# craston/object_detection_cib

Hardware: AMD Instinct MI355X
Metric: images/sec YOLOv5s 640px train (higher is better)
Workload: dtype bf16; 1 GPU; yv5s coco-zipf-like synthetic, 640px, bf16 storage/fp32 accumulate, batch 64/GPU, fwd+assign+loss+bwd+SGD, targets 4-30 boxes/img; global_batch=64, parallelism=dp1, launch=hipGraph replay, collectives=none, launcher=none, attempt=0

## Files before the change

### object_detection_cib_amd/csrc/conv_wgrad.hip

```cpp
#include <stdlib.h>

#include "kodhip_common.h"

namespace {

struct WgradArgs {
  const bf16_t* x;
  const bf16_t* dy;
  float* part;
  int B, Hs, Ws, ldx, xcoff, Cin;
  int Ho, Wo, M;
  int N, K, Kp;
  int KH, KW, SH, SW, PH, PW;
  int ldy, ycoff;
  int m_per_split, splits;
  int tiles_n, tiles_k;
  uint32_t magic_cin, magic_kw;
  uint32_t magic_hwo, magic_wo;
  const bf16_t* dy2;
  int n_half;
  int linear_map;
};

__device__ __forceinline__ bool wg_map(const WgradArgs& a, int bid, int tiles, int& tile, int& split) {
// ... 138 lines not shown
    if (st + 1 < nsteps) load_tile(m_begin + (st + 1) * 32);
    const unsigned char* Ys = lds + buf * STAGE;
    const unsigned char* Xs = Ys + 32 * SY;
#pragma unroll
    for (int ks = 0; ks < 2; ++ks) {
      bf16x8 yf[RN], xf[RK];
#pragma unroll
      for (int i = 0; i < RN; ++i) {
        const unsigned char* p = Ys + (ks * 16 + tr_row) * SY + ((wn * RN + i) * 32 + tr_col) * 2;
        s16x4 lo = __builtin_amdgcn_ds_read_tr16_b64_v4i16((s16x4 __attribute__((address_space(3)))*)(p));
        s16x4 hi = __builtin_amdgcn_ds_read_tr16_b64_v4i16((s16x4 __attribute__((address_space(3)))*)(p + 4 * SY));
        typedef short s16x8 __attribute__((ext_vector_type(8)));
        s16x8 t = {lo[0], lo[1], lo[2], lo[3], hi[0], hi[1], hi[2], hi[3]};
        yf[i] = __builtin_bit_cast(bf16x8, t);
      }
#pragma unroll
      for (int jj = 0; jj < RK; ++jj) {
        const unsigned char* p = Xs + (ks * 16 + tr_row) * SX + ((wk * RK + jj) * 32 + tr_col) * 2;
        s16x4 lo = __builtin_amdgcn_ds_read_tr16_b64_v4i16((s16x4 __attribute__((address_space(3)))*)(p));
        s16x4 hi = __builtin_amdgcn_ds_read_tr16_b64_v4i16((s16x4 __attribute__((address_space(3)))*)(p + 4 * SX));
        typedef short s16x8 __attribute__((ext_vector_type(8)));
        s16x8 t = {lo[0], lo[1], lo[2], lo[3], hi[0], hi[1], hi[2], hi[3]};
        xf[jj] = __builtin_bit_cast(bf16x8, t);
      }
#pragma unroll
      for (int i = 0; i < RN; ++i)
#pragma unroll
        for (int jj = 0; jj < RK; ++jj)
          acc[i][jj] = __builtin_amdgcn_mfma_f32_32x32x16_bf16(yf[i], xf[jj], acc[i][jj], 0, 0, 0);
    }
    if (st + 1 < nsteps) store_tile(buf ^ 1);
    __syncthreads();
  }

  float* slab = a.part + (size_t)split * a.N * a.Kp;
#pragma unroll
  for (int i = 0; i < RN; ++i)
#pragma unroll
    for (int jj = 0; jj < RK; ++jj) {
      int k = k0 + (wk * RK + jj) * 32 + (lane & 31);
#pragma unroll
      for (int e = 0; e < 16; ++e) {
        int n = n0 + (wn * RN + i) * 32 + 8 * (e >> 2) + 4 * (lane >> 5) + (e & 3);
        if (n < a.N && k < a.Kp) slab[(size_t)n * a.Kp + k] = acc[i][jj][e];
      }
    }
}

__host__ __device__ constexpr int swz_mask(int row_b) { return row_b % 256 == 0 ? 3 : (row_b % 128 == 0 ? 2 : 0); }
__device__ __forceinline__ int swz(int row, int mask) { return mask == 3 ? 4 * (row & 3) : (mask == 2 ? 4 * ((row >> 1) & 1) : 0); }

template <int N>
__device__ __forceinline__ void wait_vm() { asm volatile("s_waitcnt vmcnt(%0)" ::"n"(N) : "memory"); }
template <int WN, int WK, int RN, int RK, int NST, int RS, int GM>
__global__ __launch_bounds__(64 * WN * WK) void conv_wgrad_dma_kernel(WgradArgs a, uint32_t x_bytes, uint32_t dy_bytes) {
  constexpr int NW = WN * WK;
  constexpr int TNB = WN * RN * 32;
  constexpr int TKB = WK * RK * 32;
  constexpr int RBY = TNB * 2, RBX = TKB * 2;
  constexpr int NIY = RS * RBY / 1024, NIX = RS * RBX / 1024;
  constexpr int KS = RS / 16;
  constexpr int NI = NIY + NIX;
  constexpr int SLOTS = (NI + NW - 1) / NW;
  constexpr int STAGE = RS * RBY + RS * RBX;
  constexpr int MY = swz_mask(RBY), MX = swz_mask(RBX);
  static_assert((RS * RBY) % 1024 == 0 && (RS * RBX) % 1024 == 0, "tile rows must fill whole DMA instructions");
  __shared__ __attribute__((aligned(1024))) unsigned char lds[NST * STAGE];

  const int tid = threadIdx.x;
  const int lane = tid & 63;
  const int wave = __builtin_amdgcn_readfirstlane(tid >> 6);
  const int wn = wave / WK, wk = wave % WK;

  const int bid = blockIdx.x;
  const int tiles = a.tiles_n * a.tiles_k;
  int tile, split;
  if (!wg_map(a, bid, tiles, tile, split)) return;
  const int nt = tile % a.tiles_n;
  const bool half2 = a.n_half && nt >= (a.tiles_n >> 1);
  const int n0 = half2 ? a.n_half + (nt - (a.tiles_n >> 1)) * TNB : nt * TNB;
  const int ny0 = half2 ? n0 - a.n_half : n0;
  const int ny_hi = a.n_half ? a.n_half : a.N;
  const int n_hi = (a.n_half && !half2) ? a.n_half : a.N;
  const int k0 = (tile / a.tiles_n) * TKB;
  const int m_begin = split * a.m_per_split;
  int m_end = m_begin + a.m_per_split;
  if (m_end > a.M) m_end = a.M;
  const int HWo = a.Ho * a.Wo;

#if defined(__HIP_DEVICE_COMPILE__)
  __amdgpu_buffer_rsrc_t rs_x = __builtin_amdgcn_make_buffer_rsrc((void*)a.x, 0, x_bytes, 0x00020000);
  __amdgpu_buffer_rsrc_t rs_y = __builtin_amdgcn_make_buffer_rsrc((void*)(half2 ? a.dy2 : a.dy), 0, dy_bytes, 0x00020000);
#endif

  int s_row[SLOTS];
  uint32_t s_off[SLOTS];
  bool s_ok[SLOTS];
  int s_cy[SLOTS], s_cx[SLOTS];
  int my_slots = 0;
  constexpr bool pointwise = GM == 1;
  constexpr bool ROLE_STATIC = (NIY % NW == 0) && (NI % NW == 0);
#pragma unroll
  for (int i = 0; i < SLOTS; ++i) {
    const int t = wave + i * NW;
    s_row[i] = 0; s_off[i] = 0; s_ok[i] = false; s_cy[i] = s_cx[i] = 0;
    if (!ROLE_STATIC && t >= NI) continue;
    ++my_slots;
    if (ROLE_STATIC ? (i < NIY / NW) : (t < NIY)) {
      const int L = t * 1024 + lane * 16;
      const int row = L / RBY, pc = (L % RBY) >> 4;
      const int c = pc ^ swz(row, MY);
      s_row[i] = row;
      s_ok[i] = (ny0 + c * 8) < ny_hi;
      s_off[i] = (uint32_t)(((long)(m_begin + row) * a.ldy + a.ycoff + ny0 + c * 8) * 2);
    } else {
      const int L = (t - NIY) * 1024 + lane * 16;
      const int row = L / RBX, pc = (L % RBX) >> 4;
      const int c = pc ^ swz(row, MX);
      const int k = k0 + c * 8;
      const uint32_t tap = __umulhi((uint32_t)k, a.magic_cin);
      const int ci = k - (int)tap * a.Cin;
      const int kh = (a.KW == 1) ? (int)tap : (int)__umulhi(tap, a.magic_kw);
      s_row[i] = row;
      s_ok[i] = k < a.K;
      s_cy[i] = kh - a.PH; s_cx[i] = ((int)tap - kh * a.KW) - a.PW;
      s_off[i] = (uint32_t)((a.xcoff + ci) * 2);
      if (pointwise) s_off[i] = (uint32_t)(((long)(m_begin + row) * a.ldx + a.xcoff + ci) * 2);
    }
  }
  const uint32_t magic_hwo = a.magic_hwo, magic_wo = a.magic_wo;
  const uint32_t ldx2 = (uint32_t)a.ldx * 2u, ystep = (uint32_t)(RS * a.ldy * 2), xstep = (uint32_t)(RS * a.ldx * 2);

  int issued = 0;
  auto issue = [&](int stage) {
    unsigned char* Ys = lds + stage * STAGE;
    const int mb = m_begin + issued * RS;
#pragma unroll
    for (int i = 0; i < SLOTS; ++i) {
      const int t = wave + i * NW;
      if (!ROLE_STATIC && t >= NI) continue;
      const int m = mb + s_row[i];
      uint32_t vo;
      bool ok = s_ok[i] && m < m_end;
      const bool is_y = ROLE_STATIC ? (i < NIY / NW) : (t < NIY);
      if (is_y) {
        vo = s_off[i];
        s_off[i] += ystep;
      } else if (pointwise) {
        vo = s_off[i];
        s_off[i] += xstep;
      } else {
        uint32_t b = magic_hwo ? __umulhi((uint32_t)m, magic_hwo) : (uint32_t)m;
        int rem = m - (int)b * HWo;
        if (rem < 0) { rem += HWo; --b; }
        uint32_t oy = magic_wo ? __umulhi((uint32_t)rem, magic_wo) : (uint32_t)rem;
        int ox = rem - (int)oy * a.Wo;
        if (ox < 0) { ox += a.Wo; --oy; }
        const int iy = (int)oy * a.SH + s_cy[i];
        const int ix = ox * a.SW + s_cx[i];
        ok = ok && (unsigned)iy < (unsigned)a.Hs && (unsigned)ix < (unsigned)a.Ws;
        vo = (((uint32_t)b * (uint32_t)a.Hs + (uint32_t)iy) * (uint32_t)a.Ws + (uint32_t)ix) * ldx2 + s_off[i];
      }
      vo = ok ? vo : 0xFFFFFFF0u;
#if defined(__HIP_DEVICE_COMPILE__) && !defined(WG_ABL_NODMA)
      if (is_y)
        __builtin_amdgcn_raw_ptr_buffer_load_lds(rs_y, (__attribute__((address_space(3))) void*)(Ys + t * 1024), 16, vo, 0, 0, 0);
      else
        __builtin_amdgcn_raw_ptr_buffer_load_lds(rs_x, (__attribute__((address_space(3))) void*)(Ys + t * 1024), 16, vo, 0, 0, 0);
#else
      (void)vo; (void)Ys;
#endif
    }
    ++issued;
  };

  f32x16 acc[RN][RK];
#pragma unroll
  for (int i = 0; i < RN; ++i)
#pragma unroll
    for (int jj = 0; jj < RK; ++jj)
#pragma unroll
      for (int e = 0; e < 16; ++e) acc[i][jj][e] = 0.f;

  const int tr_row = 8 * (lane >> 5) + ((lane & 15) >> 2);
  const int tr_col = 16 * ((lane >> 4) & 1) + 4 * (lane & 3);
  const int sy = swz(tr_row, MY), sx = swz(tr_row, MX);
  const uint32_t lds_base = (uint32_t)(uintptr_t)(__attribute__((address_space(3))) unsigned char*)lds;
  uint32_t yoff[RN], xoff[RK];
#pragma unroll
  for (int i = 0; i < RN; ++i) {
    const int col = (wn * RN + i) * 32 + tr_col;
    yoff[i] = (uint32_t)(tr_row * RBY + (((col >> 3) ^ sy) << 4) + (col & 7) * 2);
  }
#pragma unroll
  for (int jj = 0; jj < RK; ++jj) {
    const int col = (wk * RK + jj) * 32 + tr_col;
    xoff[jj] = (uint32_t)(tr_row * RBX + (((col >> 3) ^ sx) << 4) + (col & 7) * 2);
  }

  const int nsteps = (m_end - m_begin + RS - 1) / RS;
#pragma unroll
  for (int p = 0; p < NST - 1; ++p)
    if (p < nsteps) issue(p);
  for (int st = 0; st < nsteps; ++st) {
    const int newer = nsteps - 1 - st;
    if (newer >= NST - 2) {
      if (my_slots == SLOTS) wait_vm<(NST - 2) * SLOTS>(); else wait_vm<(NST - 2) * (SLOTS - 1)>();
    } else if (newer == 1 && NST > 3) {
      if (my_slots == SLOTS) wait_vm<SLOTS>(); else wait_vm<SLOTS - 1>();
    } else {
      wait_vm<0>();
    }
    __builtin_amdgcn_s_barrier();
#ifndef WG_ABL_NOISSUE
    if (st + NST - 1 < nsteps) issue((st + NST - 1) % NST);
#endif
    const uint32_t ys = lds_base + (uint32_t)((st % NST) * STAGE);
    const uint32_t xs = ys + RS * RBY;
    s16x4 ylo[KS][RN], yhi[KS][RN], xlo[KS][RK], xhi[KS][RK];
#pragma unroll
    for (int ks = 0; ks < KS; ++ks) {
#pragma unroll
      for (int i = 0; i < RN; ++i) {
        const uint32_t p = ys + yoff[i] + (uint32_t)(ks * 16 * RBY);
        asm volatile("ds_read_b64_tr_b16 %0, %1" : "=v"(ylo[ks][i]) : "v"(p) : "memory");
        asm volatile("ds_read_b64_tr_b16 %0, %1" : "=v"(yhi[ks][i]) : "v"(p + 4 * RBY) : "memory");
      }
#pragma unroll
      for (int jj = 0; jj < RK; ++jj) {
        const uint32_t p = xs + xoff[jj] + (uint32_t)(ks * 16 * RBX);
        asm volatile("ds_read_b64_tr_b16 %0, %1" : "=v"(xlo[ks][jj]) : "v"(p) : "memory");
        asm volatile("ds_read_b64_tr_b16 %0, %1" : "=v"(xhi[ks][jj]) : "v"(p + 4 * RBX) : "memory");
      }
    }
#pragma unroll
    for (int ks = 0; ks < KS; ++ks) {
      constexpr int PER = 2 * (RN + RK);
      if (ks == KS - 1) asm volatile("s_waitcnt lgkmcnt(0)" ::: "memory");
      else if ((KS - 1 - ks) * PER >= 15) asm volatile("s_waitcnt lgkmcnt(15)" ::: "memory");
      else if (ks == KS - 2) asm volatile("s_waitcnt lgkmcnt(%0)" ::"n"(PER < 15 ? PER : 15) : "memory");
      else asm volatile("s_waitcnt lgkmcnt(%0)" ::"n"(2 * PER < 15 ? 2 * PER : 15) : "memory");
#pragma unroll
      for (int i = 0; i < RN; ++i) asm volatile("" : "+v"(ylo[ks][i]), "+v"(yhi[ks][i]));
#pragma unroll
      for (int jj = 0; jj < RK; ++jj) asm volatile("" : "+v"(xlo[ks][jj]), "+v"(xhi[ks][jj]));
      typedef short s16x8 __attribute__((ext_vector_type(8)));
      bf16x8 yf[RN], xf[RK];
#pragma unroll
      for (int i = 0; i < RN; ++i) {
        s16x8 t = {ylo[ks][i][0], ylo[ks][i][1], ylo[ks][i][2], ylo[ks][i][3], yhi[ks][i][0], yhi[ks][i][1], yhi[ks][i][2], yhi[ks][i][3]};
        yf[i] = __builtin_bit_cast(bf16x8, t);
      }
#pragma unroll
      for (int jj = 0; jj < RK; ++jj) {
        s16x8 t = {xlo[ks][jj][0], xlo[ks][jj][1], xlo[ks][jj][2], xlo[ks][jj][3], xhi[ks][jj][0], xhi[ks][jj][1], xhi[ks][jj][2], xhi[ks][jj][3]};
        xf[jj] = __builtin_bit_cast(bf16x8, t);
      }
#pragma unroll
      for (int i = 0; i < RN; ++i)
#pragma unroll
        for (int jj = 0; jj < RK; ++jj)
#ifdef WG_ABL_NOMFMA
          asm volatile("" ::"v"(yf[i]), "v"(xf[jj]));
#else
          acc[i][jj] = __builtin_amdgcn_mfma_f32_32x32x16_bf16(yf[i], xf[jj], acc[i][jj], 0, 0, 0);
#endif
    }
  }
  float* slab = a.part + (size_t)split * a.N * a.Kp;
#pragma unroll
  for (int i = 0; i < RN; ++i)
#pragma unroll
    for (int jj = 0; jj < RK; ++jj) {
      int k = k0 + (wk * RK + jj) * 32 + (lane & 31);
#pragma unroll
      for (int e = 0; e < 16; ++e) {
        int n = n0 + (wn * RN + i) * 32 + 8 * (e >> 2) + 4 * (lane >> 5) + (e & 3);
        if (n < n_hi && k < a.Kp) slab[(size_t)n * a.Kp + k] = acc[i][jj][e];
      }
    }
}

template <int WN, int RN, int WC, int NST>
__global__ __launch_bounds__(64 * WN * 3 * WC) void conv_wgrad_row3_kernel(WgradArgs a, uint32_t x_bytes, uint32_t dy_bytes) {
  constexpr int RS = 32;
  constexpr int NW = WN * 3 * WC;
  constexpr int TNB = WN * RN * 32;
  constexpr int RBY = TNB * 2;
  constexpr int RBX = 64;
  constexpr int XR = 48;
  constexpr int NIY = RS * RBY / 1024;
  constexpr int NXT = 3 * WC;
  constexpr int NIX = NXT * 3;
  constexpr int NI = NIY + NIX;
  constexpr int SLOTS = (NI + NW - 1) / NW;
  constexpr int XT_BYTES = XR * RBX;
  constexpr int STAGE = RS * RBY + NXT * XT_BYTES;
  constexpr int MY = swz_mask(RBY);
  constexpr int KS = RS / 16;
  static_assert((RS * RBY) % 1024 == 0 && XT_BYTES % 1024 == 0, "tiles must fill whole DMA instructions");
  __shared__ __attribute__((aligned(1024))) unsigned char lds[NST * STAGE];

  const int tid = threadIdx.x;
  const int lane = tid & 63;
  const int wave = __builtin_amdgcn_readfirstlane(tid >> 6);
  const int wc = wave % WC, kh = (wave / WC) % 3, wn = wave / (3 * WC);

  const int bid = blockIdx.x;
  const int tiles = a.tiles_n * a.tiles_k;
  int tile, split;
  if (!wg_map(a, bid, tiles, tile, split)) return;
  const int n0 = (tile % a.tiles_n) * TNB;
  const int c0 = (tile / a.tiles_n) * (WC * 32);
  const int m_begin = split * a.m_per_split;
  int m_end = m_begin + a.m_per_split;
  if (m_end > a.M) m_end = a.M;
  const int W = a.Ws, H = a.Hs, HW = a.Hs * a.Ws, BHW = a.B * HW;

#if defined(__HIP_DEVICE_COMPILE__)
  __amdgpu_buffer_rsrc_t rs_x = __builtin_amdgcn_make_buffer_rsrc((void*)a.x, 0, x_bytes, 0x00020000);
// ... 142 lines not shown
#pragma unroll
      for (int i = 0; i < RN; ++i) asm volatile("" : "+v"(ylo[ks][i]), "+v"(yhi[ks][i]));
#pragma unroll
      for (int kw = 0; kw < 3; ++kw) asm volatile("" : "+v"(xlo[ks][kw]), "+v"(xhi[ks][kw]));
      typedef short s16x8 __attribute__((ext_vector_type(8)));
      typedef unsigned int u32x2 __attribute__((ext_vector_type(2)));
      if ((inv0 | inv2) != 0) {
        const int sh = ks * 16 + 8 * (lane >> 5);
#pragma unroll
        for (int side = 0; side < 2; ++side) {
          const uint32_t bits = ((side == 0 ? inv0 : inv2) >> sh) & 0xFFu;
          const int kw = side == 0 ? 0 : 2;
          u32x2 lo = __builtin_bit_cast(u32x2, xlo[ks][kw]), hi = __builtin_bit_cast(u32x2, xhi[ks][kw]);
          lo[0] &= ((bits & 1u) ? 0u : 0xFFFFu) | ((bits & 2u) ? 0u : 0xFFFF0000u);
          lo[1] &= ((bits & 4u) ? 0u : 0xFFFFu) | ((bits & 8u) ? 0u : 0xFFFF0000u);
          hi[0] &= ((bits & 16u) ? 0u : 0xFFFFu) | ((bits & 32u) ? 0u : 0xFFFF0000u);
          hi[1] &= ((bits & 64u) ? 0u : 0xFFFFu) | ((bits & 128u) ? 0u : 0xFFFF0000u);
          xlo[ks][kw] = __builtin_bit_cast(s16x4, lo); xhi[ks][kw] = __builtin_bit_cast(s16x4, hi);
        }
      }
      bf16x8 yf[RN], xf[3];
#pragma unroll
      for (int i = 0; i < RN; ++i) {
        s16x8 t = {ylo[ks][i][0], ylo[ks][i][1], ylo[ks][i][2], ylo[ks][i][3], yhi[ks][i][0], yhi[ks][i][1], yhi[ks][i][2], yhi[ks][i][3]};
        yf[i] = __builtin_bit_cast(bf16x8, t);
      }
#pragma unroll
      for (int kw = 0; kw < 3; ++kw) {
        s16x8 t = {xlo[ks][kw][0], xlo[ks][kw][1], xlo[ks][kw][2], xlo[ks][kw][3], xhi[ks][kw][0], xhi[ks][kw][1], xhi[ks][kw][2], xhi[ks][kw][3]};
        xf[kw] = __builtin_bit_cast(bf16x8, t);
      }
#pragma unroll
      for (int i = 0; i < RN; ++i)
#pragma unroll
        for (int kw = 0; kw < 3; ++kw)
          acc[i][kw] = __builtin_amdgcn_mfma_f32_32x32x16_bf16(yf[i], xf[kw], acc[i][kw], 0, 0, 0);
    }
  }
  float* slab = a.part + (size_t)split * a.N * a.Kp;
  const int ch = c0 + wc * 32 + (lane & 31);
#pragma unroll
  for (int i = 0; i < RN; ++i)
#pragma unroll
    for (int kw = 0; kw < 3; ++kw) {
      const int k = (kh * 3 + kw) * a.Cin + ch;
#pragma unroll
      for (int e = 0; e < 16; ++e) {
        const int n = n0 + (wn * RN + i) * 32 + 8 * (e >> 2) + 4 * (lane >> 5) + (e & 3);
        if (n < a.N && ch < a.Cin) slab[(size_t)n * a.Kp + k] = acc[i][kw][e];
      }
    }
}

constexpr int RED_K = 32, RED_L = 8;
constexpr int RED_Q = 32;

template <int V> struct RedVec { typedef float type; };
template <> struct RedVec<4> { typedef f32x4 type; };
template <int V>
__device__ __forceinline__ typename RedVec<V>::type red_load(const float* p) {
  if constexpr (V == 4) return kod_load_once<f32x4>(p);
  else return *p;
}

__device__ __forceinline__ void wgrad_scatter(float* dst, int n, int k, int Cin, int KK, int stem, float v) {
  if (stem) {
    const int c = k & 3, dx = (k >> 2) & 1, tt = k >> 3;
    const int kh = tt / 3, kwp = tt - kh * 3;
    if (c < 3) dst[(size_t)n * 108 + c * 36 + kh * 6 + 2 * kwp + dx] = v;
  } else {
    const int tap = k / Cin;
    const int ci = k - tap * Cin;
    dst[(size_t)n * Cin * KK + ci * KK + tap] = v;
  }
}

template <int V>
__global__ __launch_bounds__(256) void wgrad_reduce_kernel(const float* part, float* grad, int splits, int Nfull, int N, int K,
                                                           int Kp, int Cin, int KK, int stem, float scale, float* grad2,
                                                           int n_first) {
  typedef typename RedVec<V>::type T;
  constexpr int RED_X = V == 4 ? RED_Q : RED_K;
  __shared__ T sm[RED_L][V == 4 ? RED_X : RED_X + 1];
  const int qx = threadIdx.x % RED_X, sl = threadIdx.x / RED_X;
  const int KV = K / V;
  const long q = (long)blockIdx.x * RED_X + qx;
  const long total = (long)N * KV;
  T s = {};
  int n = 0, k = 0;
  if (q < total) {
    n = (int)(q / KV);
    k = (int)(q - (long)n * KV) * V;
    const float* p = part + (size_t)n * Kp + k;
    const size_t slab = (size_t)Nfull * Kp;
    T s0 = s, s1 = s, s2 = s, s3 = s;
    int i = sl;
    for (; i + 3 * RED_L < splits; i += 4 * RED_L) {
      const T a0 = red_load<V>(p + (size_t)i * slab);
      const T a1 = red_load<V>(p + (size_t)(i + RED_L) * slab);
      const T a2 = red_load<V>(p + (size_t)(i + 2 * RED_L) * slab);
      const T a3 = red_load<V>(p + (size_t)(i + 3 * RED_L) * slab);
      s0 += a0; s1 += a1; s2 += a2; s3 += a3;
    }
    for (; i < splits; i += RED_L) s0 += red_load<V>(p + (size_t)i * slab);
    s = (s0 + s1) + (s2 + s3);
  }
  sm[sl][qx] = s;
  __syncthreads();
  if (sl == 0 && q < total) {
    T t = {};
#pragma unroll
    for (int i = 0; i < RED_L; ++i) t += sm[i][qx];
    float* dst = n >= n_first ? grad2 : grad;
    if (n >= n_first) n -= n_first;
    if constexpr (V == 4) {
#pragma unroll
      for (int e = 0; e < 4; ++e) wgrad_scatter(dst, n, k + e, Cin, KK, stem, t[e] * scale);
    } else {
      wgrad_scatter(dst, n, k, Cin, KK, stem, t * scale);
    }
  }
}

static int launch_wgrad_reduce(const float* part, float* grad, int splits, int Nfull, int N, int K, int Kp, int Cin, int KK,
                               int stem, float scale, float* grad2, int n_first, hipStream_t stream) {
  if (K % 4 == 0 && Kp % 4 == 0 && (reinterpret_cast<uintptr_t>(part) & 15) == 0)
    hipLaunchKernelGGL(wgrad_reduce_kernel<4>, dim3(cdiv((long)N * (K >> 2), RED_Q)), dim3(256), 0, stream, part, grad, splits, Nfull, N,
                       K, Kp, Cin, KK, stem, scale, grad2, n_first);
  else
    hipLaunchKernelGGL(wgrad_reduce_kernel<1>, dim3(cdiv((long)N * K, RED_K)), dim3(256), 0, stream, part, grad, splits, Nfull, N, K, Kp,
                       Cin, KK, stem, scale, grad2, n_first);
  KOD_LAUNCH_CHECK("wgrad_reduce");
  return KOD_OK;
}

#ifndef WG_NST
#define WG_NST 4
#endif
#ifndef WG_RS
#define WG_RS 32
#endif
constexpr int WGRAD_STAGES = WG_NST;
constexpr int WGRAD_ROWS = WG_RS;


struct WgradKnobs {
  bool dma;
  int row3;
  int slots;
  int row3_slots;
  int stem_tw;
  int stem_blocks;
};
const WgradKnobs& wgrad_knobs() {
  static const WgradKnobs k = [] {
    auto num = [](const char* e, int dflt) { return e ? atoi(e) : dflt; };
    WgradKnobs v;
    const char* mode = getenv("KODHIP_WGRAD_DMA");
    v.dma = !(mode && mode[0] == 'n');
    v.row3 = num(getenv("KODHIP_WGRAD_ROW3"), 1);
    v.slots = num(getenv("KODHIP_WGRAD_SLOTS"), 512);
    if (v.slots < 8) v.slots = 512;
    v.row3_slots = num(getenv("KODHIP_WGRAD_ROW3_SLOTS"), 3072);
    if (v.row3_slots < 96) v.row3_slots = 3072;
    v.stem_tw = num(getenv("KODHIP_STEM_BWD_TW"), 80);
    if (v.stem_tw != 80 && v.stem_tw != 160) v.stem_tw = 80;
    v.stem_blocks = num(getenv("KODHIP_STEM_BWD_BLOCKS"), 0);
    if (v.stem_blocks < 1) v.stem_blocks = 0;
    return v;
  }();
  return k;
}

bool wgrad_in_range(long x_bytes, long dy_bytes) { return x_bytes < (1l << 32) - 64 && dy_bytes < (1l << 32) - 64; }

enum WgradForm { WG_GENERIC, WG_ROW3, WG_DUAL };
struct WgradPlan {
  WgradForm form;
  int tn, tk;
  int wn, rn, wc;
  int tiles_n, tiles_k;
  int m_per_split, splits;
  bool dma;
  int Ho, Wo;
  long M, x_bytes, dy_bytes;
};

bool row3_eligible(int N, int Cin, int KH, int KW, int SH, int SW, int PH, int PW) {
  const int mode = wgrad_knobs().row3;
  if (!mode || KH != 3 || KW != 3 || SH != 1 || SW != 1 || PH != 1 || PW != 1 || Cin % 32 != 0 || N % 8 != 0) return false;
  return mode != 1 || N <= 32 || (Cin >= 256 && N <= 256);
}

void tile_shape(int N, int Kp, int* tn, int* tk) {
  *tn = N > 64 ? 128 : (N > 32 ? 64 : 32);
  if (N > 128 && N <= 192) *tn = 64;
  *tk = Kp > 64 ? 128 : (Kp > 32 ? 64 : 32);
  if (*tn == 32 && (Kp == 160 || Kp == 288)) *tk = Kp;
}

int rows_per_split(long M, int tiles, int resident_blocks) {
  int s = resident_blocks / tiles;
  const long maxs = (M + 255) / 256;
  if (s > maxs) s = (int)maxs;
  if (s < 1) s = 1;
  const int rows = cdiv(cdiv(M, s), 32) * 32;
  return rows < 32 ? 32 : rows;
}

WgradPlan wgrad_plan(int B, int H, int W, int ldx, int Cin, int N, int KH, int KW, int SH, int SW, int PH, int PW, int Kp, int ldy,
                     bool dual) {
  const WgradKnobs& kn = wgrad_knobs();
  if (dual) { KH = KW = SH = SW = 1; PH = PW = 0; }
  WgradPlan p = {};
  p.Ho = (H + 2 * PH - KH) / SH + 1; p.Wo = (W + 2 * PW - KW) / SW + 1;
  p.M = (long)B * p.Ho * p.Wo;
  p.x_bytes = (long)B * H * W * ldx * 2; p.dy_bytes = p.M * ldy * 2;
  const bool in_range = wgrad_in_range(p.x_bytes, p.dy_bytes);
  int resident;
  if (!dual && in_range && row3_eligible(N, Cin, KH, KW, SH, SW, PH, PW)) {
    p.form = WG_ROW3;
    p.wn = N <= 64 ? 1 : 2; p.rn = N <= 32 ? 1 : 2; p.wc = Cin >= 64 ? 2 : 1;
    p.tn = p.wn * p.rn * 32; p.tk = p.wc * 32;
    p.tiles_n = cdiv(N, p.tn); p.tiles_k = cdiv(Cin, p.tk);
    p.dma = true;
    resident = kn.row3_slots / (p.wn * 3 * p.wc);
  } else {
    p.form = dual ? WG_DUAL : WG_GENERIC;
    tile_shape(N, Kp, &p.tn, &p.tk);
    p.tiles_n = (dual ? 2 : 1) * cdiv(N, p.tn); p.tiles_k = cdiv(Kp, p.tk);
    p.dma = kn.dma && in_range;
    resident = kn.slots;
  }
  if (dual && !p.dma) return p;
  p.m_per_split = rows_per_split(p.M, p.tiles_n * p.tiles_k, resident);
  p.splits = cdiv(p.M, p.m_per_split);
  return p;
}

template <int WN, int WK, int RN, int RK>
int launch_cfg(WgradArgs a, const WgradPlan& p, hipStream_t stream) {
  constexpr int TNB = WN * RN * 32, TKB = WK * RK * 32;
  KOD_CHECK_ARG(p.tn == TNB && p.tk == TKB && p.tiles_k == cdiv(a.Kp, TKB) &&
                p.tiles_n == (a.n_half ? 2 * cdiv(a.n_half, TNB) : cdiv(a.N, TNB)), "conv_wgrad: plan and kernel instance disagree");
  const int grid = wg_grid(a);
  const dim3 g(grid), b(64 * WN * WK);
  if (p.dma) {
    const bool pw = a.KH == 1 && a.KW == 1 && a.SH == 1 && a.SW == 1 && a.PH == 0 && a.PW == 0;
    const uint32_t xb = (uint32_t)p.x_bytes, yb = (uint32_t)p.dy_bytes;
    if (pw) hipLaunchKernelGGL((conv_wgrad_dma_kernel<WN, WK, RN, RK, WGRAD_STAGES, WGRAD_ROWS, 1>), g, b, 0, stream, a, xb, yb);
    else hipLaunchKernelGGL((conv_wgrad_dma_kernel<WN, WK, RN, RK, WGRAD_STAGES, WGRAD_ROWS, 0>), g, b, 0, stream, a, xb, yb);
    KOD_LAUNCH_CHECK("conv_wgrad_dma");
    return KOD_OK;
  }
  hipLaunchKernelGGL((conv_wgrad_kernel<WN, WK, RN, RK>), g, b, 0, stream, a);
  KOD_LAUNCH_CHECK("conv_wgrad");
  return KOD_OK;
}

struct StemBwdArgs {
  const bf16_t* x;
  const bf16_t* dA; int lda, dacoff;
  const bf16_t* y; int ldy;
  const float* scale; const float* shift; const float* coef;
  float* part;
  int B, Hs, Wp, Ho, Wo, N;
  int tiles_per_row, tiles, tiles_per_block;
  uint32_t x_bytes, da_bytes, y_bytes;
};

__host__ __device__ constexpr int stem_prw(int TW) { return TW == 160 ? 168 : 88; }
__host__ __device__ constexpr int stem_xb(int TW) { return (6 * stem_prw(TW) * 16 + 1023) / 1024 * 1024; }

template <int TW, int NT>
__global__ __launch_bounds__(320, NT == 2 ? 3 : (TW == 160 ? 3 : 5)) void conv_stem_bwd_fused_kernel(StemBwdArgs a) {
  constexpr int PRW = stem_prw(TW), NW = 5;
  constexpr int CH = 4 * NT, RBG = 64 * NT;
  constexpr int XB = stem_xb(TW), GB = TW * RBG;
  constexpr int STAGE = XB + 2 * GB;
  constexpr int NIX = XB / 1024, NIG = GB / 1024, NI = NIX + 2 * NIG;
  constexpr int ITEMS = TW * CH / 320;
  static_assert(GB % 1024 == 0 && TW * CH % 320 == 0 && 320 % CH == 0, "tile must fill whole DMA instructions / thread items");
  __shared__ __attribute__((aligned(1024))) unsigned char lds[2 * STAGE];
  const int tid = threadIdx.x, lane = tid & 63;
  const int wave = __builtin_amdgcn_readfirstlane(tid >> 6);
  const int t_begin = blockIdx.x * a.tiles_per_block;
  int t_end = t_begin + a.tiles_per_block;
  if (t_end > a.tiles) t_end = a.tiles;

#if defined(__HIP_DEVICE_COMPILE__)
  __amdgpu_buffer_rsrc_t rs_x = __builtin_amdgcn_make_buffer_rsrc((void*)a.x, 0, a.x_bytes, 0x00020000);
  __amdgpu_buffer_rsrc_t rs_g = __builtin_amdgcn_make_buffer_rsrc((void*)a.dA, 0, a.da_bytes, 0x00020000);
  __amdgpu_buffer_rsrc_t rs_y = __builtin_amdgcn_make_buffer_rsrc((void*)a.y, 0, a.y_bytes, 0x00020000);
#endif

  const int cc = tid % CH;
  float sc[8], sh[8], k1[8], k2[8], k3[8];
#pragma unroll
  for (int e = 0; e < 8; ++e) {
    const int c = cc * 8 + e;
    const bool ok = c < a.N;
    sc[e] = ok ? a.scale[c] : 0.f; sh[e] = ok ? a.shift[c] : 0.f;
    k1[e] = ok ? a.coef[c] : 0.f; k2[e] = ok ? a.coef[a.N + c] : 0.f; k3[e] = ok ? a.coef[2 * a.N + c] : 0.f;
  }
// ... 78 lines not shown
#pragma unroll
      for (int e = 0; e < 8; ++e) {
        const float yv = (float)y8[e];
        const float z = __builtin_fmaf(yv, sc[e], sh[e]);
        const float sg = kod_sigmoid_l2(KOD_NEG_LOG2E * z);
        const float dz = kod_silu_bwd((float)g8[e], z, sg);
        o[e] = (bf16_t)__builtin_fmaf(k1[e], dz, __builtin_fmaf(k2[e], yv, k3[e]));
      }
      if (!(ch_ok && ox0 + p < a.Wo)) o = bf16x8{};
      const u32x4 ov = __builtin_bit_cast(u32x4, o);
      asm volatile("ds_write_b128 %0, %1" ::"v"(ga), "v"(ov) : "memory");
    }
    asm volatile("s_waitcnt lgkmcnt(0)" ::: "memory");
    __builtin_amdgcn_s_barrier();

#pragma unroll 2
    for (int ks = 0; ks < TW / 16; ++ks) {
      s16x4 ylo[NT], yhi[NT], xlo, xhi;
      const uint32_t px = sb + xoff + (uint32_t)(ks * 16 * 16);
#pragma unroll
      for (int n = 0; n < NT; ++n) {
        const uint32_t py = sb + yoff + (uint32_t)(ks * 16 * RBG + n * 64);
        asm volatile("ds_read_b64_tr_b16 %0, %1" : "=v"(ylo[n]) : "v"(py) : "memory");
        asm volatile("ds_read_b64_tr_b16 %0, %1" : "=v"(yhi[n]) : "v"(py + 4 * RBG) : "memory");
      }
      asm volatile("ds_read_b64_tr_b16 %0, %1" : "=v"(xlo) : "v"(px) : "memory");
      asm volatile("ds_read_b64_tr_b16 %0, %1" : "=v"(xhi) : "v"(px + 4 * 16) : "memory");
      asm volatile("s_waitcnt lgkmcnt(0)" ::: "memory");
      asm volatile("" : "+v"(xlo), "+v"(xhi));
      typedef short s16x8 __attribute__((ext_vector_type(8)));
      const s16x8 tx = {xlo[0], xlo[1], xlo[2], xlo[3], xhi[0], xhi[1], xhi[2], xhi[3]};
#pragma unroll
      for (int n = 0; n < NT; ++n) {
        asm volatile("" : "+v"(ylo[n]), "+v"(yhi[n]));
        const s16x8 ty = {ylo[n][0], ylo[n][1], ylo[n][2], ylo[n][3], yhi[n][0], yhi[n][1], yhi[n][2], yhi[n][3]};
        acc[n] = __builtin_amdgcn_mfma_f32_32x32x16_bf16(__builtin_bit_cast(bf16x8, ty), __builtin_bit_cast(bf16x8, tx), acc[n], 0, 0, 0);
      }
    }
    buf ^= 1;
  }

  float* slab = a.part + (size_t)blockIdx.x * (32 * NT) * 160;
  const int k = wave * 32 + (lane & 31);
#pragma unroll
  for (int nt = 0; nt < NT; ++nt)
#pragma unroll
    for (int e = 0; e < 16; ++e) {
      const int n = nt * 32 + 8 * (e >> 2) + 4 * (lane >> 5) + (e & 3);
      slab[(size_t)n * 160 + k] = acc[nt][e];
    }
}

template <int WN, int RN, int WC>
int launch_row3(WgradArgs a, const WgradPlan& p, hipStream_t stream) {
  constexpr int NST = (WN * 3 * WC == 3 || (WN == 1 && RN == 2 && WC == 2)) ? 3 : 4;
  KOD_CHECK_ARG(p.tiles_n == cdiv(a.N, WN * RN * 32) && p.tiles_k == cdiv(a.Cin, WC * 32), "conv_wgrad: plan and ROW3 instance disagree");
  const int grid = wg_grid(a);
  hipLaunchKernelGGL((conv_wgrad_row3_kernel<WN, RN, WC, NST>), dim3(grid), dim3(64 * WN * 3 * WC), 0, stream, a, (uint32_t)p.x_bytes,
                     (uint32_t)p.dy_bytes);
  KOD_LAUNCH_CHECK("conv_wgrad_row3");
  return KOD_OK;
}

typedef int (*WgradLaunch)(WgradArgs, const WgradPlan&, hipStream_t);
struct WgradTile { int tn, tk; WgradLaunch launch; };
const WgradTile WGRAD_TILES[] = {
    {128, 128, launch_cfg<2, 2, 2, 2>}, {64, 128, launch_cfg<2, 2, 1, 2>}, {32, 160, launch_cfg<1, 5, 1, 1>},
    {32, 288, launch_cfg<1, 9, 1, 1>},  {32, 128, launch_cfg<1, 4, 1, 1>}, {128, 64, launch_cfg<2, 2, 2, 1>},
    {64, 64, launch_cfg<2, 2, 1, 1>},   {32, 64, launch_cfg<1, 2, 1, 1>},  {128, 32, launch_cfg<4, 1, 1, 1>},
    {64, 32, launch_cfg<2, 1, 1, 1>},   {32, 32, launch_cfg<1, 1, 1, 1>},
};
struct WgradRow3 { int wn, rn, wc; WgradLaunch launch; };
const WgradRow3 WGRAD_ROW3[] = {
    {1, 1, 1, launch_row3<1, 1, 1>}, {1, 1, 2, launch_row3<1, 1, 2>}, {1, 2, 1, launch_row3<1, 2, 1>},
    {1, 2, 2, launch_row3<1, 2, 2>}, {2, 2, 1, launch_row3<2, 2, 1>}, {2, 2, 2, launch_row3<2, 2, 2>},
};

int wgrad_partial(WgradArgs& a, const char* who, const void* x, const void* dy, const void* dy2, float* partials, int B, int H, int W,
                  int ldx, int xcoff, int Cin, int N, int KH, int KW, int SH, int SW, int PH, int PW, int Kp, int ldy, int ycoff,
                  hipStream_t stream) {
  const bool dual = dy2 != nullptr;
  KOD_CHECK_ARG(x && dy && partials, "%s: null pointer", who);
  KOD_CHECK_ARG(Cin % 8 == 0 && ldx % 8 == 0 && xcoff % 8 == 0 && xcoff + Cin <= ldx, "%s: bad input slice", who);
  KOD_CHECK_ARG(N % 8 == 0 && ldy % 8 == 0 && ycoff % 8 == 0 && ycoff + N <= ldy, "%s: bad dy slice (N=%d ldy=%d)", who, N, ldy);
  KOD_CHECK_ARG(Kp % 32 == 0 && Kp >= KH * KW * Cin, "%s: bad Kp", who);
  const WgradPlan p = wgrad_plan(B, H, W, ldx, Cin, N, KH, KW, SH, SW, PH, PW, Kp, ldy, dual);
  KOD_CHECK_ARG(p.M < (1l << 31) && (long)B * H * W < (1l << 31), "%s: pixel count overflows int32", who);
  KOD_CHECK_ARG(p.splits > 0, "%s: not available for this geometry (kodhip_conv_wgrad_dual_splits == 0)", who);
  a = WgradArgs{};
  a.x = (const bf16_t*)x; a.dy = (const bf16_t*)dy; a.dy2 = (const bf16_t*)dy2; a.part = partials;
  a.B = B; a.Hs = H; a.Ws = W; a.ldx = ldx; a.xcoff = xcoff; a.Cin = Cin;
  a.Ho = p.Ho; a.Wo = p.Wo; a.M = (int)p.M;
  a.N = dual ? 2 * N : N; a.n_half = dual ? N : 0; a.K = KH * KW * Cin; a.Kp = Kp;
  a.KH = KH; a.KW = KW; a.SH = SH; a.SW = SW; a.PH = PH; a.PW = PW; a.ldy = ldy; a.ycoff = ycoff;
  a.magic_cin = magic_u32((uint32_t)Cin); a.magic_kw = magic_u32((uint32_t)KW);
  a.magic_hwo = magic_u32((uint32_t)(a.Ho * a.Wo)); a.magic_wo = magic_u32((uint32_t)a.Wo);
  a.m_per_split = p.m_per_split; a.splits = p.splits;
  a.tiles_n = p.tiles_n; a.tiles_k = p.tiles_k;
  if (p.form == WG_ROW3) {
    for (const WgradRow3& r : WGRAD_ROW3)
      if (r.wn == p.wn && r.rn == p.rn && r.wc == p.wc) return r.launch(a, p, stream);
  } else {
    for (const WgradTile& t : WGRAD_TILES)
      if (t.tn == p.tn && t.tk == p.tk) return t.launch(a, p, stream);
  }
  KOD_CHECK_ARG(false, "%s: no kernel instance for the plan's tile %d x %d", who, p.tn, p.tk);
  return KOD_EARG;
}

struct StemBwdPlan { int TW, tiles_per_row, tiles, blocks, tiles_per_block, slab_rows; };
StemBwdPlan stem_bwd_plan(int B, int H, int Wp, int N) {
  const WgradKnobs& kn = wgrad_knobs();
  StemBwdPlan p;
  p.TW = (N > 32 || Wp <= 80) ? 80 : kn.stem_tw;
  p.tiles_per_row = cdiv(Wp, p.TW);
  const long tiles = (long)B * (H / 2) * p.tiles_per_row;
  const int want = kn.stem_blocks ? kn.stem_blocks : (N > 32 ? 512 : (p.TW == 160 ? 512 : 1024));
// ... 82 lines not shown
```

### object_detection_cib_amd/engine/options.py

```python
from __future__ import annotations

import dataclasses
import os
from dataclasses import dataclass, field
from typing import Dict

NATIVE_KNOBS = ("KODHIP_NO_FAST", "KODHIP_FORCE_BM", "KODHIP_FORCE_BN", "KODHIP_S2_SEPARATE", "KODHIP_S2_FOLD_MAXC",
                "KODHIP_ROW3", "KODHIP_WGRAD_DMA", "KODHIP_WGRAD_SLOTS", "KODHIP_WGRAD_ROW3", "KODHIP_WGRAD_ROW3_SLOTS",
                "KODHIP_STEM_BWD_BLOCKS", "KODHIP_STEM_BWD_TW", "KODHIP_STEM_BWD_STREAM", "KODHIP_DEBUG_STAMPS", "KODHIP_LIB",
                "KODHIP_BN_U", "KODHIP_BN_GRID", "KODHIP_BN_BLOCK", "KODHIP_BN_LDS")


def _flag(name: str, default: bool) -> bool:
    v = os.environ.get(name)
    if v is None:
        return default
    return v not in ("0", "", "false", "False")


@dataclass
class EngineOptions:
    wgrad_overlap: bool = True
    branch_overlap: bool = True
    comm_overlap: bool = True
    force_collectives: bool = False
    syncbn_exchange: str = "auto"
    dual_dgrad: bool = True
    bn_reduce_fused: bool = True
    bn_reduce_min_k: int = 0
    dx_accum_fp32: bool = False
    dual_wgrad: bool = True
    stem_bwd_fused: bool = True
    eval_fused: bool = False
    debug_plan: bool = False
    max_shape_sets: int = 4
    bucket_mb: float = 8.0
    native: Dict[str, str] = field(default_factory=dict)

    @staticmethod
    def from_env() -> "EngineOptions":
        e = os.environ
        return EngineOptions(
            wgrad_overlap=_flag("KODHIP_WGRAD_OVERLAP", True),
            branch_overlap=_flag("KODHIP_BRANCH_OVERLAP", True),
            comm_overlap=_flag("KODHIP_COMM_OVERLAP", True),
            force_collectives=_flag("KODHIP_FORCE_COLLECTIVES", False),
            syncbn_exchange=e.get("KODHIP_SYNCBN", "auto"),
            dual_dgrad=not _flag("KODHIP_NO_DUAL", False),
            bn_reduce_fused=not _flag("KODHIP_NO_BNRED", False),
            bn_reduce_min_k=int(e.get("KODHIP_BNRED_MINK", "0")),
            dx_accum_fp32=_flag("KODHIP_DX_FP32", False),
            dual_wgrad=not _flag("KODHIP_NO_DUAL_WGRAD", False),
            stem_bwd_fused=_flag("KODHIP_STEM_BWD_FUSED", True),
            eval_fused=_flag("KODHIP_EVAL_FUSED", False),
            debug_plan=_flag("KODHIP_DEBUG_PLAN", False),
            max_shape_sets=int(e.get("KODHIP_MAX_SHAPE_SETS", "4")),
            native={k: e[k] for k in NATIVE_KNOBS if k in e},
        )

    def as_dict(self) -> dict:
        return dataclasses.asdict(self)
# ... 1 lines not shown
```

Before: 5659 images/sec.

## Add two-group wgrad blocks with in-LDS accumulator merge and chain-parallel split reduce

```diff
diff --git a/object_detection_cib_amd/csrc/conv_wgrad.hip b/object_detection_cib_amd/csrc/conv_wgrad.hip
--- a/object_detection_cib_amd/csrc/conv_wgrad.hip
+++ b/object_detection_cib_amd/csrc/conv_wgrad.hip
@@ -214,25 +214,30 @@
 
 template <int N>
 __device__ __forceinline__ void wait_vm() { asm volatile("s_waitcnt vmcnt(%0)" ::"n"(N) : "memory"); }
-template <int WN, int WK, int RN, int RK, int NST, int RS, int GM>
-__global__ __launch_bounds__(64 * WN * WK) void conv_wgrad_dma_kernel(WgradArgs a, uint32_t x_bytes, uint32_t dy_bytes) {
-  constexpr int NW = WN * WK;
+template <int WN, int WK, int RN, int RK, int NST, int RS, int GM, int G>
+__global__ __launch_bounds__(64 * WN * WK * G) void conv_wgrad_dma_kernel(WgradArgs a, uint32_t x_bytes, uint32_t dy_bytes) {
+  constexpr int NWG = WN * WK;
+  constexpr int NW = NWG * G;
+  constexpr int RSS = RS * G;
   constexpr int TNB = WN * RN * 32;
   constexpr int TKB = WK * RK * 32;
   constexpr int RBY = TNB * 2, RBX = TKB * 2;
-  constexpr int NIY = RS * RBY / 1024, NIX = RS * RBX / 1024;
+  constexpr int NIY = RSS * RBY / 1024, NIX = RSS * RBX / 1024;
   constexpr int KS = RS / 16;
   constexpr int NI = NIY + NIX;
   constexpr int SLOTS = (NI + NW - 1) / NW;
-  constexpr int STAGE = RS * RBY + RS * RBX;
+  constexpr int STAGE = RSS * RBY + RSS * RBX;
   constexpr int MY = swz_mask(RBY), MX = swz_mask(RBX);
-  static_assert((RS * RBY) % 1024 == 0 && (RS * RBX) % 1024 == 0, "tile rows must fill whole DMA instructions");
+  static_assert((RSS * RBY) % 1024 == 0 && (RSS * RBX) % 1024 == 0, "tile rows must fill whole DMA instructions");
+  static_assert(G == 1 || (G == 2 && NST * STAGE >= NWG * RN * RK * 16 * 64 * 4), "the ring must hold group 1's accumulators");
+  static_assert(NST * STAGE <= 160 * 1024 && 64 * NW <= 1024, "block beyond a CU");
   __shared__ __attribute__((aligned(1024))) unsigned char lds[NST * STAGE];
 
   const int tid = threadIdx.x;
   const int lane = tid & 63;
   const int wave = __builtin_amdgcn_readfirstlane(tid >> 6);
-  const int wn = wave / WK, wk = wave % WK;
+  const int grp = wave / NWG, wl = wave % NWG;
+  const int wn = wl / WK, wk = wl % WK;
 
   const int bid = blockIdx.x;
   const int tiles = a.tiles_n * a.tiles_k;
@@ -291,12 +296,12 @@
     }
   }
   const uint32_t magic_hwo = a.magic_hwo, magic_wo = a.magic_wo;
-  const uint32_t ldx2 = (uint32_t)a.ldx * 2u, ystep = (uint32_t)(RS * a.ldy * 2), xstep = (uint32_t)(RS * a.ldx * 2);
+  const uint32_t ldx2 = (uint32_t)a.ldx * 2u, ystep = (uint32_t)(RSS * a.ldy * 2), xstep = (uint32_t)(RSS * a.ldx * 2);
 
   int issued = 0;
   auto issue = [&](int stage) {
     unsigned char* Ys = lds + stage * STAGE;
-    const int mb = m_begin + issued * RS;
+    const int mb = m_begin + issued * RSS;
 #pragma unroll
     for (int i = 0; i < SLOTS; ++i) {
       const int t = wave + i * NW;
@@ -352,15 +357,15 @@
 #pragma unroll
   for (int i = 0; i < RN; ++i) {
     const int col = (wn * RN + i) * 32 + tr_col;
-    yoff[i] = (uint32_t)(tr_row * RBY + (((col >> 3) ^ sy) << 4) + (col & 7) * 2);
+    yoff[i] = (uint32_t)((grp * RS + tr_row) * RBY + (((col >> 3) ^ sy) << 4) + (col & 7) * 2);
   }
 #pragma unroll
   for (int jj = 0; jj < RK; ++jj) {
     const int col = (wk * RK + jj) * 32 + tr_col;
-    xoff[jj] = (uint32_t)(tr_row * RBX + (((col >> 3) ^ sx) << 4) + (col & 7) * 2);
-  }
-
-  const int nsteps = (m_end - m_begin + RS - 1) / RS;
+    xoff[jj] = (uint32_t)((grp * RS + tr_row) * RBX + (((col >> 3) ^ sx) << 4) + (col & 7) * 2);
+  }
+
+  const int nsteps = (m_end - m_begin + RSS - 1) / RSS;
 #pragma unroll
   for (int p = 0; p < NST - 1; ++p)
     if (p < nsteps) issue(p);
@@ -378,7 +383,7 @@
     if (st + NST - 1 < nsteps) issue((st + NST - 1) % NST);
 #endif
     const uint32_t ys = lds_base + (uint32_t)((st % NST) * STAGE);
-    const uint32_t xs = ys + RS * RBY;
+    const uint32_t xs = ys + RSS * RBY;
     s16x4 ylo[KS][RN], yhi[KS][RN], xlo[KS][RK], xhi[KS][RK];
 #pragma unroll
     for (int ks = 0; ks < KS; ++ks) {
@@ -428,6 +433,26 @@
           acc[i][jj] = __builtin_amdgcn_mfma_f32_32x32x16_bf16(yf[i], xf[jj], acc[i][jj], 0, 0, 0);
 #endif
     }
+  }
+  if constexpr (G == 2) {
+    __syncthreads();
+    float* ex = reinterpret_cast<float*>(lds) + wl * (RN * RK * 16 * 64) + lane;
+    if (grp == 1) {
+#pragma unroll
+      for (int i = 0; i < RN; ++i)
+#pragma unroll
+        for (int jj = 0; jj < RK; ++jj)
+#pragma unroll
+          for (int e = 0; e < 16; ++e) ex[((i * RK + jj) * 16 + e) * 64] = acc[i][jj][e];
+    }
+    __syncthreads();
+    if (grp == 1) return;
+#pragma unroll
+    for (int i = 0; i < RN; ++i)
+#pragma unroll
+      for (int jj = 0; jj < RK; ++jj)
+#pragma unroll
+        for (int e = 0; e < 16; ++e) acc[i][jj][e] = acc[i][jj][e] + ex[((i * RK + jj) * 16 + e) * 64];
   }
   float* slab = a.part + (size_t)split * a.N * a.Kp;
 #pragma unroll
@@ -676,8 +701,11 @@
     }
 }
 
-constexpr int RED_K = 32, RED_L = 8;
-constexpr int RED_Q = 32;
+constexpr int RED_L = 8;
+constexpr int RED_F = 8;
+constexpr int RED_ONE_CHAIN = 3 * RED_L;
+constexpr int RED_X4 = 8;
+constexpr long RED_NARROW = 256;
 
 template <int V> struct RedVec { typedef float type; };
 template <> struct RedVec<4> { typedef f32x4 type; };
@@ -699,14 +727,15 @@
   }
 }
 
-template <int V>
-__global__ __launch_bounds__(256) void wgrad_reduce_kernel(const float* part, float* grad, int splits, int Nfull, int N, int K,
+template <int V, int C, int RED_X>
+__global__ __launch_bounds__(RED_X * RED_L * C) void wgrad_reduce_kernel(const float* part, float* grad, int splits, int Nfull, int N, int K,
                                                            int Kp, int Cin, int KK, int stem, float scale, float* grad2,
                                                            int n_first) {
   typedef typename RedVec<V>::type T;
-  constexpr int RED_X = V == 4 ? RED_Q : RED_K;
-  __shared__ T sm[RED_L][V == 4 ? RED_X : RED_X + 1];
-  const int qx = threadIdx.x % RED_X, sl = threadIdx.x / RED_X;
+  static_assert(C == 1 || C == 4, "a thread per lane or a thread per chain");
+  __shared__ T sm[RED_L * C][V == 4 ? RED_X : RED_X + 1];
+  const int qx = threadIdx.x % RED_X, ch = threadIdx.x / RED_X;
+  const int sl = ch / C, j = ch % C;
   const int KV = K / V;
   const long q = (long)blockIdx.x * RED_X + qx;
   const long total = (long)N * KV;
@@ -715,26 +744,55 @@
   if (q < total) {
     n = (int)(q / KV);
     k = (int)(q - (long)n * KV) * V;
-    const float* p = part + (size_t)n * Kp + k;
     const size_t slab = (size_t)Nfull * Kp;
-    T s0 = s, s1 = s, s2 = s, s3 = s;
-    int i = sl;
-    for (; i + 3 * RED_L < splits; i += 4 * RED_L) {
-      const T a0 = red_load<V>(p + (size_t)i * slab);
-      const T a1 = red_load<V>(p + (size_t)(i + RED_L) * slab);
-      const T a2 = red_load<V>(p + (size_t)(i + 2 * RED_L) * slab);
-      const T a3 = red_load<V>(p + (size_t)(i + 3 * RED_L) * slab);
-      s0 += a0; s1 += a1; s2 += a2; s3 += a3;
-    }
-    for (; i < splits; i += RED_L) s0 += red_load<V>(p + (size_t)i * slab);
-    s = (s0 + s1) + (s2 + s3);
-  }
-  sm[sl][qx] = s;
+    const float* p0 = part + (size_t)n * Kp + k;
+    constexpr int ROUND = 4 * RED_L;
+    if constexpr (C == 4) {
+      const int left = splits - 3 * RED_L - sl;
+      const int rounds = left > 0 ? (left + ROUND - 1) / ROUND : 0;
+      const float* p = p0 + (size_t)(sl + j * RED_L) * slab;
+      const size_t step = (size_t)ROUND * slab;
+      for (int t = 0; t < rounds; t += RED_F) {
+        T a[RED_F];
+#pragma unroll
+        for (int u = 0; u < RED_F; ++u)
+          if (t + u < rounds) a[u] = red_load<V>(p + (size_t)(t + u) * step);
+#pragma unroll
+        for (int u = 0; u < RED_F; ++u)
+          if (t + u < rounds) s += a[u];
+      }
+      if (j == 0) {
+        T a[3];
+#pragma unroll
+        for (int u = 0; u < 3; ++u)
+          if (sl + rounds * ROUND + u * RED_L < splits) a[u] = red_load<V>(p0 + (size_t)(sl + rounds * ROUND + u * RED_L) * slab);
+#pragma unroll
+        for (int u = 0; u < 3; ++u)
+          if (sl + rounds * ROUND + u * RED_L < splits) s += a[u];
+      }
+    } else {
+      T s1 = s, s2 = s, s3 = s;
+      int i = sl;
+      for (; i + 3 * RED_L < splits; i += ROUND) {
+        const T a0 = red_load<V>(p0 + (size_t)i * slab);
+        const T a1 = red_load<V>(p0 + (size_t)(i + RED_L) * slab);
+        const T a2 = red_load<V>(p0 + (size_t)(i + 2 * RED_L) * slab);
+        const T a3 = red_load<V>(p0 + (size_t)(i + 3 * RED_L) * slab);
+        s += a0; s1 += a1; s2 += a2; s3 += a3;
+      }
+      for (; i < splits; i += RED_L) s += red_load<V>(p0 + (size_t)i * slab);
+      s = (s + s1) + (s2 + s3);
+    }
+  }
+  sm[ch][qx] = s;
   __syncthreads();
-  if (sl == 0 && q < total) {
+  if (ch == 0 && q < total) {
     T t = {};
 #pragma unroll
-    for (int i = 0; i < RED_L; ++i) t += sm[i][qx];
+    for (int i = 0; i < RED_L; ++i) {
+      if constexpr (C == 4) t += (sm[4 * i][qx] + sm[4 * i + 1][qx]) + (sm[4 * i + 2][qx] + sm[4 * i + 3][qx]);
+      else t += sm[i][qx];
+    }
     float* dst = n >= n_first ? grad2 : grad;
     if (n >= n_first) n -= n_first;
     if constexpr (V == 4) {
@@ -746,14 +804,22 @@
   }
 }
 
+template <int V, int C>
+static void launch_wgrad_reduce_as(long quads, hipStream_t stream, const float* part, float* grad, int splits, int Nfull, int N, int K,
+                                   int Kp, int Cin, int KK, int stem, float scale, float* grad2, int n_first) {
+  constexpr int X = C == 1 ? 32 : RED_X4;
+  hipLaunchKernelGGL((wgrad_reduce_kernel<V, C, X>), dim3(cdiv(quads, X)), dim3(X * RED_L * C), 0, stream, part, grad, splits, Nfull,
+                     N, K, Kp, Cin, KK, stem, scale, grad2, n_first);
+}
+
 static int launch_wgrad_reduce(const float* part, float* grad, int splits, int Nfull, int N, int K, int Kp, int Cin, int KK,
                                int stem, float scale, float* grad2, int n_first, hipStream_t stream) {
-  if (K % 4 == 0 && Kp % 4 == 0 && (reinterpret_cast<uintptr_t>(part) & 15) == 0)
-    hipLaunchKernelGGL(wgrad_reduce_kernel<4>, dim3(cdiv((long)N * (K >> 2), RED_Q)), dim3(256), 0, stream, part, grad, splits, Nfull, N,
-                       K, Kp, Cin, KK, stem, scale, grad2, n_first);
-  else
-    hipLaunchKernelGGL(wgrad_reduce_kernel<1>, dim3(cdiv((long)N * K, RED_K)), dim3(256), 0, stream, part, grad, splits, Nfull, N, K, Kp,
-                       Cin, KK, stem, scale, grad2, n_first);
+  const bool v4 = K % 4 == 0 && Kp % 4 == 0 && (reinterpret_cast<uintptr_t>(part) & 15) == 0;
+  const long quads = v4 ? (long)N * (K >> 2) : (long)N * K;
+  const bool one = splits <= RED_ONE_CHAIN || cdiv(quads, 32) >= RED_NARROW;
+  auto* go = v4 ? (one ? launch_wgrad_reduce_as<4, 1> : launch_wgrad_reduce_as<4, 4>)
+                : (one ? launch_wgrad_reduce_as<1, 1> : launch_wgrad_reduce_as<1, 4>);
+  go(quads, stream, part, grad, splits, Nfull, N, K, Kp, Cin, KK, stem, scale, grad2, n_first);
   KOD_LAUNCH_CHECK("wgrad_reduce");
   return KOD_OK;
 }
@@ -775,6 +841,7 @@
   int row3_slots;
   int stem_tw;
   int stem_blocks;
+  int groups;
 };
 const WgradKnobs& wgrad_knobs() {
   static const WgradKnobs k = [] {
@@ -791,6 +858,8 @@
     if (v.stem_tw != 80 && v.stem_tw != 160) v.stem_tw = 80;
     v.stem_blocks = num(getenv("KODHIP_STEM_BWD_BLOCKS"), 0);
     if (v.stem_blocks < 1) v.stem_blocks = 0;
+    v.groups = num(getenv("KODHIP_WGRAD_GROUPS"), 0);
+    if (v.groups < 0 || v.groups > 2) v.groups = 0;
     return v;
   }();
   return k;
@@ -863,17 +932,30 @@
 }
 
 template <int WN, int WK, int RN, int RK>
-int launch_cfg(WgradArgs a, const WgradPlan& p, hipStream_t stream) {
+int launch_cfg(WgradArgs& a, const WgradPlan& p, hipStream_t stream) {
   constexpr int TNB = WN * RN * 32, TKB = WK * RK * 32;
+  constexpr bool HAS_TWO = 2 * WN * WK <= 16 && WGRAD_STAGES * 2 * WGRAD_ROWS * (TNB + TKB) * 2 <= 160 * 1024;
+  const bool pw = a.KH == 1 && a.KW == 1 && a.SH == 1 && a.SW == 1 && a.PH == 0 && a.PW == 0;
+  const int groups = wgrad_knobs().groups;
+  const bool two = HAS_TWO && p.dma && p.splits >= 2 && (groups == 2 || (groups == 0 && pw));
+  if (two) { a.m_per_split = 2 * p.m_per_split; a.splits = cdiv(p.splits, 2); }
   KOD_CHECK_ARG(p.tn == TNB && p.tk == TKB && p.tiles_k == cdiv(a.Kp, TKB) &&
                 p.tiles_n == (a.n_half ? 2 * cdiv(a.n_half, TNB) : cdiv(a.N, TNB)), "conv_wgrad: plan and kernel instance disagree");
   const int grid = wg_grid(a);
   const dim3 g(grid), b(64 * WN * WK);
   if (p.dma) {
-    const bool pw = a.KH == 1 && a.KW == 1 && a.SH == 1 && a.SW == 1 && a.PH == 0 && a.PW == 0;
     const uint32_t xb = (uint32_t)p.x_bytes, yb = (uint32_t)p.dy_bytes;
-    if (pw) hipLaunchKernelGGL((conv_wgrad_dma_kernel<WN, WK, RN, RK, WGRAD_STAGES, WGRAD_ROWS, 1>), g, b, 0, stream, a, xb, yb);
-    else hipLaunchKernelGGL((conv_wgrad_dma_kernel<WN, WK, RN, RK, WGRAD_STAGES, WGRAD_ROWS, 0>), g, b, 0, stream, a, xb, yb);
+    if constexpr (HAS_TWO) {
+      if (two) {
+        const dim3 b2(2 * 64 * WN * WK);
+        if (pw) hipLaunchKernelGGL((conv_wgrad_dma_kernel<WN, WK, RN, RK, WGRAD_STAGES, WGRAD_ROWS, 1, 2>), g, b2, 0, stream, a, xb, yb);
+        else hipLaunchKernelGGL((conv_wgrad_dma_kernel<WN, WK, RN, RK, WGRAD_STAGES, WGRAD_ROWS, 0, 2>), g, b2, 0, stream, a, xb, yb);
+        KOD_LAUNCH_CHECK("conv_wgrad_dma");
+        return KOD_OK;
+      }
+    }
+    if (pw) hipLaunchKernelGGL((conv_wgrad_dma_kernel<WN, WK, RN, RK, WGRAD_STAGES, WGRAD_ROWS, 1, 1>), g, b, 0, stream, a, xb, yb);
+    else hipLaunchKernelGGL((conv_wgrad_dma_kernel<WN, WK, RN, RK, WGRAD_STAGES, WGRAD_ROWS, 0, 1>), g, b, 0, stream, a, xb, yb);
     KOD_LAUNCH_CHECK("conv_wgrad_dma");
     return KOD_OK;
   }
@@ -1058,7 +1140,7 @@
 }
 
 template <int WN, int RN, int WC>
-int launch_row3(WgradArgs a, const WgradPlan& p, hipStream_t stream) {
+int launch_row3(WgradArgs& a, const WgradPlan& p, hipStream_t stream) {
   constexpr int NST = (WN * 3 * WC == 3 || (WN == 1 && RN == 2 && WC == 2)) ? 3 : 4;
   KOD_CHECK_ARG(p.tiles_n == cdiv(a.N, WN * RN * 32) && p.tiles_k == cdiv(a.Cin, WC * 32), "conv_wgrad: plan and ROW3 instance disagree");
   const int grid = wg_grid(a);
@@ -1068,7 +1150,7 @@
   return KOD_OK;
 }
 
-typedef int (*WgradLaunch)(WgradArgs, const WgradPlan&, hipStream_t);
+typedef int (*WgradLaunch)(WgradArgs&, const WgradPlan&, hipStream_t);
 struct WgradTile { int tn, tk; WgradLaunch launch; };
 const WgradTile WGRAD_TILES[] = {
     {128, 128, launch_cfg<2, 2, 2, 2>}, {64, 128, launch_cfg<2, 2, 1, 2>}, {32, 160, launch_cfg<1, 5, 1, 1>},
diff --git a/object_detection_cib_amd/engine/options.py b/object_detection_cib_amd/engine/options.py
--- a/object_detection_cib_amd/engine/options.py
+++ b/object_detection_cib_amd/engine/options.py
@@ -7,6 +7,7 @@
 
 NATIVE_KNOBS = ("KODHIP_NO_FAST", "KODHIP_FORCE_BM", "KODHIP_FORCE_BN", "KODHIP_S2_SEPARATE", "KODHIP_S2_FOLD_MAXC",
                 "KODHIP_ROW3", "KODHIP_WGRAD_DMA", "KODHIP_WGRAD_SLOTS", "KODHIP_WGRAD_ROW3", "KODHIP_WGRAD_ROW3_SLOTS",
+                "KODHIP_WGRAD_GROUPS",
                 "KODHIP_STEM_BWD_BLOCKS", "KODHIP_STEM_BWD_TW", "KODHIP_STEM_BWD_STREAM", "KODHIP_DEBUG_STAMPS", "KODHIP_LIB",
                 "KODHIP_BN_U", "KODHIP_BN_GRID", "KODHIP_BN_BLOCK", "KODHIP_BN_LDS")
 
```

Result: no change. 5697 images/sec, median of 6 (+0.7%).
